# joshbeal/mira

Measured on AMD Instinct MI355X. Metric: bn256_g1_msm_throughput, higher is better.
Workload: dtype u256 mod p (9 x 29-bit limbs in u32/u64, Montgomery)

## Files before the change

mira_amd/csrc/msm_host.cuh:

```cuda
#pragma once
#include "ctx.h"
#ifndef MSM_DIGITS_BLOCK
#define MSM_DIGITS_BLOCK 256
#endif
#include "msm_kernels.cuh"
#include "table_kernels.cuh"
#include "sort_kernels.cuh"
#include "reduce_kernels.cuh"
#include "host_field.hpp"
#include <cerrno>
#include <thread>
#include <unistd.h>

#ifdef MIRA_CPU_EMU
static constexpr uint32_t FIXUP_HEAVY_GRID = 4;
static constexpr uint32_t FIXUP_HEAVY_BLOCKS = 1;
#else
#ifndef MIRA_FIXUP_HEAVY_BLOCKS
#define MIRA_FIXUP_HEAVY_BLOCKS 256
#endif
static constexpr uint32_t FIXUP_HEAVY_BLOCKS = MIRA_FIXUP_HEAVY_BLOCKS;
static constexpr uint32_t FIXUP_HEAVY_GRID = 1024;
#endif

static constexpr uint32_t SCAN_OWN_PREFIX_TILES = 32;
static constexpr uint32_t SCAN_SOLO_TILES = 2;
static inline bool reduce_with_quads(uint64_t work_items) { return work_items * 4 <= 98304; }
#ifdef MIRA_CPU_EMU
static constexpr uint32_t SET_FINISH_BLOCK = 32;
#else
static constexpr uint32_t SET_FINISH_BLOCK = 256;
#endif

static inline std::vector<size_t> host_chunks(size_t n, size_t min_n) {
    std::vector<size_t> ends;
    if (n < min_n) { ends.push_back(n); return ends; }
    size_t done = 0, step = std::max<size_t>(1, min_n / 2);
    while (done < n) {
        size_t len = std::min(step, n - done);
        if (n - done - len < step / 2) len = n - done;
        done += len;
        ends.push_back(done);
        if (step < 4 * std::max<size_t>(1, min_n / 2)) step <<= 1;
    }
    return ends;
}

template <class F, class FS>
static int msm_launch_body(const Bases &bs, size_t first, const void *d_scalars, const void *h_scalars, size_t n, const MsmPlan &p,
                           uint64_t *host_windows );
template <class F, class FS>
static int msm_launch(const Bases &bs, size_t first, const void *d_scalars, const void *h_scalars, size_t n, const MsmPlan &p,
                      uint64_t *host_windows) {
    const uint32_t hist_sel_before = g.hist_sel;
    const int rc = msm_launch_body<F, FS>(bs, first, d_scalars, h_scalars, n, p, host_windows);
    if (rc != MIRA_OK) {
        if (g.copy_stream) (void)rt_sync(g.copy_stream);
        (void)rt_sync(g.stream);
        (void)rt_last();
        if (p.stats && g.hist_dev.p) {
            (void)rt_memset(g.hist_dev.p, 0, 2048, g.stream);
            (void)rt_sync(g.stream);
            g.hist_sel = hist_sel_before;
        }
    }
    return rc;
}
template <class F, class FS>
static int msm_launch_body(const Bases &bs, size_t first, const void *d_scalars, const void *h_scalars, size_t n, const MsmPlan &p,
                           uint64_t *host_windows ) {
    int rc;
    const size_t mult = p.glv ? 2 : 1;
    const size_t host_min = tuned(MIRA_TUNE_HOST_CHUNK_MIN_N, (size_t)1 << 19);
    std::vector<size_t> ends;
    if (h_scalars && p.count == 1) ends = host_chunks(n, host_min);
    else if (p.h_batch) {
        for (size_t e : host_chunks(n * p.count, host_min)) ends.push_back(std::min(n, (e + p.count - 1) / p.count));
        ends.back() = n;
        ends.erase(std::unique(ends.begin(), ends.end()), ends.end());
    } else ends = {n};
    {
        const uint64_t pass_entries = (1ull << tuned(MIRA_TUNE_PASS_ENTRIES_LOG, 32)) - 1;
        const size_t max_chunk = std::max<size_t>(64, (size_t)(pass_entries / ((uint64_t)mult * p.Wt)) / 64 * 64);
        std::vector<size_t> cut;
        for (size_t k = 0, lo = 0; k < ends.size(); lo = ends[k++])
            for (size_t at = lo; at < ends[k];) { at = std::min(ends[k], at + max_chunk); cut.push_back(at); }
        ends.swap(cut);
    }
    size_t nmax = 0;
    for (size_t k = 0, lo = 0; k < ends.size(); lo = ends[k++]) nmax = std::max(nmax, ends[k] - lo);
    nmax *= mult;
    const size_t entries_max = nmax * p.Wt;
    if ((rc = g.digits.ensure(entries_max * 2))) return rc;
    if ((rc = g.counts.ensure(((size_t)p.NB + 1) * 4))) return rc;
    if ((rc = g.offsets.ensure(((size_t)p.NB + 1) * 4))) return rc;
    if ((rc = g.cursor.ensure(((size_t)p.NB + 1) * 4))) return rc;
    const uint32_t scan_blocks = ceil_div(p.NB, SCAN_TILE);
    if (scan_blocks > 1024) { set_error("window configuration exceeds the scan capacity"); return MIRA_E_UNSUPPORTED; }
    if ((rc = g.block_sums.ensure(1024 * 4))) return rc;
    if ((rc = g.sorted_idx.ensure(entries_max * 4 + 8))) return rc;
    const size_t staged_min_n = tuned(MIRA_TUNE_STAGED_MIN_N, (size_t)1 << 19);
    if (nmax * p.count >= staged_min_n && p.c >= 9) {
        if ((rc = g.part.ensure(entries_max * 8 + 8))) return rc;
        if ((rc = g.coarse_offsets.ensure(((size_t)p.Wt * 512 + 1) * 4))) return rc;
    }
    if ((rc = g.bucket_sums.ensure((size_t)p.NB * XYZZ29_BYTES))) return rc;
    if ((rc = g.head_part.ensure((size_t)p.T * XYZZ29_BYTES))) return rc;
    if ((rc = g.tail_part.ensure((size_t)p.T * XYZZ29_BYTES))) return rc;
    if ((rc = g.tail_key.ensure((size_t)p.T * 4))) return rc;
    if ((rc = g.heavy.ensure(64 + ((size_t)p.T / 2 + 8) * 32 + ((size_t)p.T / 4 + 8) * 16))) return rc;
    if ((rc = g.heavy_out.ensure(((size_t)p.T / 2 + 8) * XYZZ29_BYTES))) return rc;
    const size_t node_points = ((size_t)p.nsets << p.gamma) * (p.kappa + 2);
    if ((rc = g.chunks.ensure(node_points * XYZZ29_BYTES))) return rc;
    if ((rc = g.window_sums.ensure((size_t)p.nsets * p.pieces * 128 + 1024))) return rc;
#ifndef MIRA_CPU_EMU
    if (h_scalars || p.h_batch) {
        if (!g.copy_stream) RT_CHECK(hipStreamCreateWithFlags(&g.copy_stream, hipStreamNonBlocking));
        while (g.copy_events.size() < ends.size()) {
            hipEvent_t e;
            RT_CHECK(hipEventCreateWithFlags(&e, hipEventDisableTiming));
            g.copy_events.push_back(e);
        }
    }
#endif

    hipStream_t st = g.stream;
    uint32_t *heavy_count = reinterpret_cast<uint32_t *>(g.heavy.p);
    U4 *heavy_runs = reinterpret_cast<U4 *>(heavy_count + 16);
    U4 *heavy_subs = heavy_runs + ((size_t)p.T / 4 + 4);
    U4 *heavy_meds = reinterpret_cast<U4 *>(reinterpret_cast<unsigned char *>(g.heavy.p) + 64 + ((size_t)p.T / 2 + 8) * 32);
    uint32_t *plan = heavy_count + 2;
    uint32_t *no_u32 = nullptr;
    unsigned char *no_u8 = nullptr;
    const uint32_t fine_bits = (p.c - 1) - std::min<uint32_t>(p.c - 1, 8);
    const uint32_t CB = p.B >> fine_bits;

    tm_begin();
    uint32_t *hist = nullptr, *hist_clear = nullptr;
    if (p.stats) {
        if (!g.hist_dev.p) {
            if ((rc = g.hist_dev.ensure(2048))) return rc;
            RT_CHECK(rt_memset(g.hist_dev.p, 0, 2048, st));
            g.hist_sel = 0;
        }
        hist = reinterpret_cast<uint32_t *>(g.hist_dev.p) + 256 * g.hist_sel;
        hist_clear = reinterpret_cast<uint32_t *>(g.hist_dev.p) + 256 * (g.hist_sel ^ 1u);
        g.hist_sel ^= 1u;
    }
    for (size_t k = 0, lo = 0; k < ends.size(); lo = ends[k++]) {
        const size_t ns = ends[k] - lo, nc = ns * mult, entries = nc * p.Wt;
        const unsigned char *sc = reinterpret_cast<const unsigned char *>(d_scalars) + (p.h_batch ? lo * p.count : lo) * 32;
        const uint64_t stride_k = p.h_batch ? (uint64_t)ns : (uint64_t)p.stride;
        const unsigned char *bases = p.shared ? reinterpret_cast<const unsigned char *>(p.shared_tables)
                                   : p.glv  ? reinterpret_cast<const unsigned char *>(p.glv_bases) + (first + lo) * 128
                                            : reinterpret_cast<const unsigned char *>(bs.d) + (first + lo) * 64;
        const uint32_t wgroup = p.shared ? p.W : 1u, idx_stride = p.shared ? (uint32_t)p.table_n : 0u, idx_first = p.shared ? (uint32_t)(first + lo) : 0u;
        const uint32_t add = k ? 1u : 0u;
        if (h_scalars || p.h_batch) {
            hipStream_t cs = g.copy_stream ? g.copy_stream : st;
            if (p.h_batch)
                for (uint32_t b = 0; b < p.count; b++)
                    RT_CHECK(rt_h2d(const_cast<unsigned char *>(sc) + (size_t)b * ns * 32, reinterpret_cast<const unsigned char *>(p.h_batch[b]) + lo * 32, ns * 32, cs));
            else
                RT_CHECK(rt_h2d(const_cast<unsigned char *>(sc), reinterpret_cast<const unsigned char *>(h_scalars) + lo * 32, ns * 32, cs));
            if (cs != st) RT_CHECK(rt_stream_wait(st, cs, g.copy_events[k]));
        }
        const uint32_t tile = (std::max<uint32_t>(1024, ceil_div(nc, std::max<uint32_t>(1, MSM_HIST_WGS / p.Wt))) + 1023) / 1024 * 1024, ntiles = ceil_div(nc, tile);
        const bool staged = nc * p.count >= staged_min_n && p.c >= 9;
        if (p.glv)
            LAUNCH((k_digits<FS, true>), dim3(ceil_div(ns, MSM_DIGITS_BLOCK), p.count), MSM_DIGITS_BLOCK, 0, st, sc, (uint32_t)ns, stride_k, p.c, p.W,
                   reinterpret_cast<int16_t *>(g.digits.p), reinterpret_cast<uint32_t *>(g.counts.p), p.NB + 1, hist, hist_clear);
        else
        LAUNCH(k_digits<FS>, dim3(ceil_div(nc, MSM_DIGITS_BLOCK), p.count), MSM_DIGITS_BLOCK, 0, st, sc, (uint32_t)nc, stride_k, p.c, p.W,
               reinterpret_cast<int16_t *>(g.digits.p), reinterpret_cast<uint32_t *>(g.counts.p), p.NB + 1, hist, hist_clear);
        tm_mark("digits");
        LAUNCH_BARRIER_FLEX(k_hist, dim3(ntiles, p.Wt), 1024, (size_t)p.B * 4, st, reinterpret_cast<const int16_t *>(g.digits.p), (uint32_t)nc,
                       p.B, tile, reinterpret_cast<uint32_t *>(g.counts.p), wgroup);
        tm_mark("hist");
        if (scan_blocks <= SCAN_SOLO_TILES) {
            LAUNCH_BARRIER(k_scan_c<SCAN_SOLO>, 1, SCAN_BLOCK, 0, st, reinterpret_cast<const uint32_t *>(g.counts.p), p.NB,
                           reinterpret_cast<const uint32_t *>(g.block_sums.p), reinterpret_cast<uint32_t *>(g.offsets.p),
                           reinterpret_cast<uint32_t *>(g.cursor.p), staged ? reinterpret_cast<uint32_t *>(g.coarse_offsets.p) : no_u32, fine_bits,
                           plan, p.lanes, p.L, heavy_count, add ? no_u8 : reinterpret_cast<unsigned char *>(g.bucket_sums.p));
        } else if (scan_blocks <= SCAN_OWN_PREFIX_TILES) {
            LAUNCH_BARRIER(k_scan_c<SCAN_OWN_PREFIX>, scan_blocks, SCAN_BLOCK, 0, st, reinterpret_cast<const uint32_t *>(g.counts.p), p.NB,
                           reinterpret_cast<const uint32_t *>(g.block_sums.p), reinterpret_cast<uint32_t *>(g.offsets.p),
                           reinterpret_cast<uint32_t *>(g.cursor.p), staged ? reinterpret_cast<uint32_t *>(g.coarse_offsets.p) : no_u32, fine_bits,
                           plan, p.lanes, p.L, heavy_count, add ? no_u8 : reinterpret_cast<unsigned char *>(g.bucket_sums.p));
        } else {
        LAUNCH_BARRIER(k_scan_a, scan_blocks, SCAN_BLOCK, 0, st, reinterpret_cast<const uint32_t *>(g.counts.p), p.NB,
                       reinterpret_cast<uint32_t *>(g.block_sums.p));
        LAUNCH_BARRIER(k_scan_b, 1, 1024, 0, st, reinterpret_cast<uint32_t *>(g.block_sums.p), scan_blocks);
        LAUNCH_BARRIER(k_scan_c<SCAN_BLOCK_SUMS>, scan_blocks, SCAN_BLOCK, 0, st, reinterpret_cast<const uint32_t *>(g.counts.p), p.NB,
                       reinterpret_cast<const uint32_t *>(g.block_sums.p), reinterpret_cast<uint32_t *>(g.offsets.p),
                       reinterpret_cast<uint32_t *>(g.cursor.p), staged ? reinterpret_cast<uint32_t *>(g.coarse_offsets.p) : no_u32, fine_bits,
                       plan, p.lanes, p.L, heavy_count, add ? no_u8 : reinterpret_cast<unsigned char *>(g.bucket_sums.p));
        }
        tm_mark("scan");
        if (staged) {
            if (p.shared)
                LAUNCH_BARRIER((k_stage1<int16_t, true, STAGE_TILE_PW>), dim3(ceil_div(nc, STAGE_TILE_PW), p.Wt), 1024, (size_t)STAGE_TILE_PW * 8, st, reinterpret_cast<const int16_t *>(g.digits.p),
                                    (uint32_t)nc, p.B, fine_bits, CB, idx_stride, idx_first, wgroup, reinterpret_cast<uint32_t *>(g.coarse_offsets.p), reinterpret_cast<U2 *>(g.part.p));
            else
                LAUNCH_BARRIER((k_stage1<int16_t, false, STAGE_TILE_PW>), dim3(ceil_div(nc, STAGE_TILE_PW), p.Wt), 1024, (size_t)STAGE_TILE_PW * 8, st, reinterpret_cast<const int16_t *>(g.digits.p),
                                    (uint32_t)nc, p.B, fine_bits, CB, 0u, 0u, 1u, reinterpret_cast<uint32_t *>(g.coarse_offsets.p), reinterpret_cast<U2 *>(g.part.p));
            tm_mark("sort_level1");
            LAUNCH_BARRIER((k_stage2<STAGE_TILE_PW, STAGE_MAX_KEYS2_PW>), ceil_div(entries, STAGE_TILE_PW), 1024, (size_t)STAGE_TILE_PW * 6, st, reinterpret_cast<const U2 *>(g.part.p),
                                reinterpret_cast<const uint32_t *>(g.offsets.p) + p.NB, fine_bits, reinterpret_cast<uint32_t *>(g.cursor.p),
                                reinterpret_cast<uint32_t *>(g.sorted_idx.p));
        } else
            LAUNCH_BARRIER_FLEX(k_scatter, dim3(ntiles, p.Wt), 1024, (size_t)p.B * 4, st, reinterpret_cast<const int16_t *>(g.digits.p),
                       (uint32_t)nc, p.B, tile, reinterpret_cast<uint32_t *>(g.cursor.p), reinterpret_cast<uint32_t *>(g.sorted_idx.p), wgroup, idx_stride, idx_first);
        tm_mark("scatter");
        if (add)
            LAUNCH((k_accumulate<F, true>), ceil_div(p.T, 128), 128, 0, st, reinterpret_cast<const uint32_t *>(g.sorted_idx.p),
                   reinterpret_cast<const uint32_t *>(g.offsets.p), p.NB, bases, (const uint32_t *)plan,
                   reinterpret_cast<unsigned char *>(g.bucket_sums.p), reinterpret_cast<unsigned char *>(g.head_part.p),
                   reinterpret_cast<unsigned char *>(g.tail_part.p), reinterpret_cast<uint32_t *>(g.tail_key.p), heavy_count, heavy_runs, heavy_subs, heavy_meds);
        else
            LAUNCH((k_accumulate<F, false>), ceil_div(p.T, 128), 128, 0, st, reinterpret_cast<const uint32_t *>(g.sorted_idx.p),
                   reinterpret_cast<const uint32_t *>(g.offsets.p), p.NB, bases, (const uint32_t *)plan,
                   reinterpret_cast<unsigned char *>(g.bucket_sums.p), reinterpret_cast<unsigned char *>(g.head_part.p),
                   reinterpret_cast<unsigned char *>(g.tail_part.p), reinterpret_cast<uint32_t *>(g.tail_key.p), heavy_count, heavy_runs, heavy_subs, heavy_meds);
        tm_mark("accumulate");
        const uint32_t fix_by_bucket = p.NB < p.T ? p.NB : 0u;
        const uint32_t fix_items = fix_by_bucket ? fix_by_bucket : p.T;
        LAUNCH_BARRIER(k_fixup_all<F>, FIXUP_HEAVY_BLOCKS + ceil_div(fix_items, HEAVY_BLOCK_A / 4), HEAVY_BLOCK_A, 0, st, FIXUP_HEAVY_BLOCKS, (const uint32_t *)plan,
                       reinterpret_cast<const uint32_t *>(g.offsets.p), reinterpret_cast<const unsigned char *>(g.head_part.p), reinterpret_cast<const unsigned char *>(g.tail_part.p),
                       reinterpret_cast<const uint32_t *>(g.tail_key.p), reinterpret_cast<unsigned char *>(g.bucket_sums.p), fix_by_bucket,
                       (const uint32_t *)heavy_count, (const U4 *)heavy_subs, (const U4 *)heavy_runs, reinterpret_cast<unsigned char *>(g.heavy_out.p), (const U4 *)heavy_meds);
        LAUNCH_BARRIER(k_fixup_heavy_b<F>, (FIXUP_HEAVY_GRID + 3) / 4, HEAVY_BLOCK_B, 0, st, (const uint32_t *)heavy_count, (const U4 *)heavy_runs,
                       reinterpret_cast<const unsigned char *>(g.heavy_out.p), reinterpret_cast<const unsigned char *>(g.tail_part.p),
                       reinterpret_cast<unsigned char *>(g.bucket_sums.p));
        tm_mark("fixup");
    }
    PieceCfg pc;
    pc.P = p.pieces;
    for (uint32_t i = 0; i <= 8; i++) pc.start[i] = piece_start(p.cb, p.pieces, std::min(i, p.pieces));
    const uint32_t tree_groups = p.nsets << p.gamma, npts = p.nsets * p.pieces;
    const size_t lds_a = ((size_t)2 << p.kappa) * XYZZ29_BYTES, lds_b = ((size_t)(p.kappa + 2) << p.gamma) * XYZZ29_BYTES;
    if (p.rquad)
        LAUNCH_BARRIER((k_bucket_tree<F, true>), tree_groups, std::max(4u, 4u << p.kappa), lds_a, st, reinterpret_cast<const unsigned char *>(g.bucket_sums.p),
                       p.lambda, p.kappa, reinterpret_cast<unsigned char *>(g.chunks.p));
    else
        LAUNCH_BARRIER((k_bucket_tree<F, false>), tree_groups, std::max(4u, 1u << p.kappa), lds_a, st, reinterpret_cast<const unsigned char *>(g.bucket_sums.p),
                       p.lambda, p.kappa, reinterpret_cast<unsigned char *>(g.chunks.p));
    tm_mark("reduce_chunks");
    uint32_t *no_ctr = nullptr;
    uint64_t *no_flag = nullptr;
    if (g.windows_dst) {
        LAUNCH_BARRIER(k_set_finish<F>, p.nsets, SET_FINISH_BLOCK, lds_b, st, reinterpret_cast<const unsigned char *>(g.chunks.p), p.kappa + 2, p.gamma, p.lambda, pc,
                       reinterpret_cast<unsigned char *>(g.window_sums.p), (const uint32_t *)hist, no_ctr, no_flag, (uint64_t)0);
        tm_mark("window_sum");
        RT_CHECK(rt_last());
        RT_CHECK(rt_d2d(g.windows_dst, g.window_sums.p, (size_t)npts * 128, st));
        RT_CHECK(rt_sync(st));
    } else {
        const size_t bytes = (size_t)npts * 128 + 1024, flag_at = (bytes + 63) / 64 * 64;
        if (g.out_host_cap < flag_at + 64) {
            RT_CHECK(rt_sync(st));
            if (g.out_host) (void)rt_host_free(g.out_host);
            g.out_host = g.out_host_dev = nullptr; g.out_host_cap = 0;
            RT_CHECK(rt_host_alloc_mapped(reinterpret_cast<void **>(&g.out_host), reinterpret_cast<void **>(&g.out_host_dev), flag_at + 64 + 4096));
            g.out_host_cap = flag_at + 64 + 4096;
        }
        if (!g.finish_ctr.p) {
            if ((rc = g.finish_ctr.ensure(64))) return rc;
            RT_CHECK(rt_memset(g.finish_ctr.p, 0, 64, st));
        }
        uint64_t *flag_host = reinterpret_cast<uint64_t *>(g.out_host + flag_at);
        const uint64_t stamp = ++g.out_stamp;
        __atomic_store_n(flag_host, (uint64_t)0, __ATOMIC_RELEASE);
        LAUNCH_BARRIER(k_set_finish<F>, p.nsets, SET_FINISH_BLOCK, lds_b, st, reinterpret_cast<const unsigned char *>(g.chunks.p), p.kappa + 2, p.gamma, p.lambda, pc,
                       g.out_host_dev, (const uint32_t *)hist, reinterpret_cast<uint32_t *>(g.finish_ctr.p), reinterpret_cast<uint64_t *>(g.out_host_dev + flag_at), stamp);
        tm_mark("window_sum");
        RT_CHECK(rt_last());
        if (g.tm.enabled || (size_t)n * p.count > ((size_t)1 << 21)) RT_CHECK(rt_sync(st));
        RT_CHECK(rt_wait_flag(flag_host, stamp, st));
        memcpy(host_windows, g.out_host, (size_t)npts * 128);
        if (p.stats) memcpy(g.hist_host, g.out_host + (size_t)npts * 128, 1024);
    }
    tm_end();
    return MIRA_OK;
}


template <class F, class FS> static int curve_init() {
#ifndef MIRA_CPU_EMU
    RT_CHECK(hipFuncSetAttribute(reinterpret_cast<const void *>(k_window_sum<F, false>), hipFuncAttributeMaxDynamicSharedMemorySize, 160 * 1024));
    RT_CHECK(hipFuncSetAttribute(reinterpret_cast<const void *>(k_bucket_tree<F, true>), hipFuncAttributeMaxDynamicSharedMemorySize, 160 * 1024));
    RT_CHECK(hipFuncSetAttribute(reinterpret_cast<const void *>(k_bucket_tree<F, false>), hipFuncAttributeMaxDynamicSharedMemorySize, 160 * 1024));
    RT_CHECK(hipFuncSetAttribute(reinterpret_cast<const void *>(k_set_finish<F>), hipFuncAttributeMaxDynamicSharedMemorySize, 160 * 1024));
    RT_CHECK(hipFuncSetAttribute(reinterpret_cast<const void *>(k_hist), hipFuncAttributeMaxDynamicSharedMemorySize, 160 * 1024));
    RT_CHECK(hipFuncSetAttribute(reinterpret_cast<const void *>(k_scatter), hipFuncAttributeMaxDynamicSharedMemorySize, 160 * 1024));
    RT_CHECK(hipFuncSetAttribute(reinterpret_cast<const void *>(k_stage1<int16_t, false, STAGE_TILE_PW>), hipFuncAttributeMaxDynamicSharedMemorySize, STAGE_TILE_PW * 8));
    RT_CHECK(hipFuncSetAttribute(reinterpret_cast<const void *>(k_stage1<int32_t, true>), hipFuncAttributeMaxDynamicSharedMemorySize, STAGE_TILE * 8));
    RT_CHECK(hipFuncSetAttribute(reinterpret_cast<const void *>(k_stage1<int16_t, true, STAGE_TILE_PW>), hipFuncAttributeMaxDynamicSharedMemorySize, STAGE_TILE_PW * 8));
    RT_CHECK(hipFuncSetAttribute(reinterpret_cast<const void *>(k_stage2<STAGE_TILE, STAGE_MAX_KEYS2>), hipFuncAttributeMaxDynamicSharedMemorySize, STAGE_TILE * 6));
    RT_CHECK(hipFuncSetAttribute(reinterpret_cast<const void *>(k_stage2<STAGE_TILE_PW, STAGE_MAX_KEYS2_PW>), hipFuncAttributeMaxDynamicSharedMemorySize, STAGE_TILE_PW * 6));
#endif
    return MIRA_OK;
}
template <class FS> static int synth_scalars(size_t n, uint64_t index0, uint64_t seed, int kind, void *d_out) {
    LAUNCH(k_synth_scalars<FS>, ceil_div(n, 256), 256, 0, g.stream, (uint64_t)n, index0, seed, kind, reinterpret_cast<unsigned char *>(d_out));
    RT_CHECK(rt_last());
    RT_CHECK(rt_sync(g.stream));
    return MIRA_OK;
}
template <class FB, int CURVE> static int synth_bases(size_t n, uint64_t index0, uint64_t seed, void *d_out) {
    LAUNCH(k_synth_bases<FB>, ceil_div(n, 64), 64, 0, g.stream, (uint64_t)n, index0, seed, reinterpret_cast<const unsigned char *>(dev_consts()->gen[CURVE]),
           reinterpret_cast<unsigned char *>(d_out));
    RT_CHECK(rt_last());
    RT_CHECK(rt_sync(g.stream));
    return MIRA_OK;
}
template <class F, int CURVE> static int check_bases(const Bases &bs, uint32_t *d_bad) {
    LAUNCH(k_check_on_curve<F>, ceil_div(bs.n, 256), 256, 0, g.stream, (const unsigned char *)bs.d, (uint64_t)bs.n,
           reinterpret_cast<const unsigned char *>(dev_consts()->b_r261[CURVE]), d_bad);
    RT_CHECK(rt_last());
    return MIRA_OK;
}
template <class F> static int convert_bases(const void *d_src, void *d_dst, size_t n) {
    if (!n) return MIRA_OK;
    LAUNCH(k_convert_bases<F>, ceil_div(n, 256), 256, 0, g.stream, reinterpret_cast<const unsigned char *>(d_src),
           reinterpret_cast<unsigned char *>(d_dst), (uint64_t)n);
    RT_CHECK(rt_last());
    RT_CHECK(rt_sync(g.stream));
    return MIRA_OK;
}
template <class F> static int export_bases(const Bases &bs, size_t first, size_t n, void *d_out) {
    if (!n) return MIRA_OK;
    LAUNCH(k_export_bases<F>, ceil_div(n, 256), 256, 0, g.stream, reinterpret_cast<const unsigned char *>(bs.d) + first * 64,
           reinterpret_cast<unsigned char *>(d_out), (uint64_t)n);
    RT_CHECK(rt_last());
    RT_CHECK(rt_sync(g.stream));
    return MIRA_OK;
}

template <class F, int CURVE> static int build_glv(Bases &bs) {
    const size_t bytes = (size_t)bs.n * 128;
    void *t = nullptr;
    if (rt_malloc(&t, bytes) != hipSuccess || !t) {
        set_error("device allocation of " + std::to_string(bytes) + " bytes for the endomorphism copy of the key failed");
        return MIRA_E_ALLOC;
    }
    LAUNCH(k_glv_bases<F>, ceil_div(bs.n, 256), 256, 0, g.stream, reinterpret_cast<const unsigned char *>(bs.d), reinterpret_cast<unsigned char *>(t), (uint64_t)bs.n,
           reinterpret_cast<const unsigned char *>(dev_consts()->beta_r261[CURVE]));
    if (rt_last() != hipSuccess || rt_sync(g.stream) != hipSuccess) { (void)rt_free(t); set_error("building the endomorphism copy of the key failed"); return MIRA_E_NO_DEVICE; }
    bs.glv = t;
    return MIRA_OK;
}

template <class F> static int build_tables(Bases &bs, uint32_t c, uint32_t W) {
    if (bs.tables || bs.n == 0) return MIRA_OK;
    const size_t bytes = (size_t)W * bs.n * 64;
    void *t = nullptr;
    if (rt_malloc(&t, bytes) != hipSuccess || !t) {
        set_error("device allocation of " + std::to_string(bytes) + " bytes for the window tables failed");
        return MIRA_E_ALLOC;
    }
    unsigned char *tb = reinterpret_cast<unsigned char *>(t);
    RT_CHECK(rt_d2d(tb, bs.d, bs.n * 64, g.stream));
    for (uint32_t w = 1; w < W; w++)
        LAUNCH(k_table_step<F>, ceil_div(bs.n, 64), 64, 0, g.stream, (const unsigned char *)(tb + (size_t)(w - 1) * bs.n * 64),
               tb + (size_t)w * bs.n * 64, (uint64_t)bs.n, c);
    RT_CHECK(rt_last());
    RT_CHECK(rt_sync(g.stream));
    bs.tables = t; bs.table_c = c; bs.table_w = W;
    return MIRA_OK;
}

template <class F, class FS>
static int msm_launch_table(const Bases &bs, size_t first, const void *d_scalars, size_t n, uint64_t *host_sums) {
    int rc;
    const TableCfg tc = table_cfg(bs.table_c);
    const uint32_t TABLE_W = tc.W, TABLE_B = tc.B, TABLE_FINE_BITS = tc.fine_bits;
    const size_t entries = (size_t)n * TABLE_W;
    const uint32_t lanes = 256u * 4u * 3u * 64u, Lmin = 16;
    const uint32_t T = (uint32_t)std::min<uint64_t>(lanes, ceil_div(entries, Lmin));
    const uint32_t m = 8, nchunks = TABLE_B / m;
    if ((rc = g.digits.ensure(entries * 4))) return rc;
    if ((rc = g.counts.ensure(((size_t)TABLE_CB + 1) * 4))) return rc;
    if ((rc = g.coarse_offsets.ensure(((size_t)TABLE_CB + 1) * 4))) return rc;
    if ((rc = g.cursor.ensure(((size_t)TABLE_CB + 1) * 4))) return rc;
    if ((rc = g.block_sums.ensure(1024 * 4))) return rc;
    if ((rc = g.part.ensure(entries * 8 + 8))) return rc;
    if ((rc = g.sorted_idx.ensure(entries * 4 + 8))) return rc;
    if ((rc = g.offsets.ensure(((size_t)TABLE_B + 1) * 4))) return rc;
    if ((rc = g.fine_counts.ensure(((size_t)TABLE_B + 1) * 4))) return rc;
    if ((rc = g.fine_cursor.ensure(((size_t)TABLE_B + 1) * 4))) return rc;
    if ((rc = g.bucket_sums.ensure((size_t)TABLE_B * XYZZ29_BYTES))) return rc;
    if ((rc = g.head_part.ensure((size_t)T * XYZZ29_BYTES))) return rc;
    if ((rc = g.tail_part.ensure((size_t)T * XYZZ29_BYTES))) return rc;
    if ((rc = g.tail_key.ensure((size_t)T * 4))) return rc;
    if ((rc = g.heavy.ensure(64 + ((size_t)T / 2 + 8) * 32 + ((size_t)T / 4 + 8) * 16))) return rc;
    if ((rc = g.heavy_out.ensure(((size_t)T / 2 + 8) * XYZZ29_BYTES))) return rc;
    if ((rc = g.chunks.ensure((size_t)nchunks * XYZZ29_BYTES))) return rc;
    if ((rc = g.window_sums.ensure((size_t)TABLE_SUMS * 128))) return rc;

    hipStream_t st = g.stream;
    uint32_t *heavy_count = reinterpret_cast<uint32_t *>(g.heavy.p);
    uint32_t *plan = heavy_count + 2;
    U4 *heavy_runs = reinterpret_cast<U4 *>(heavy_count + 16);
    U4 *heavy_subs = heavy_runs + ((size_t)T / 4 + 4);
    U4 *heavy_meds = reinterpret_cast<U4 *>(reinterpret_cast<unsigned char *>(g.heavy.p) + 64 + ((size_t)T / 2 + 8) * 32);
    const uint32_t tile = 32768, ntiles = ceil_div(n, tile);
    tm_begin();
    uint32_t *no_u32 = nullptr;
    unsigned char *no_u8 = nullptr;
    RT_CHECK(rt_memset(g.counts.p, 0, ((size_t)TABLE_CB + 1) * 4, st));
    tm_mark("memset");
    LAUNCH(k_digits32<FS>, ceil_div(n, 256), 256, 0, st, reinterpret_cast<const unsigned char *>(d_scalars), (uint32_t)n, tc.c, tc.W,
           reinterpret_cast<int32_t *>(g.digits.p));
    tm_mark("digits");
    LAUNCH_BARRIER_FLEX(k_thist_coarse, dim3(ntiles, TABLE_W), 512, 0, st, reinterpret_cast<const int32_t *>(g.digits.p), (uint32_t)n, tile, TABLE_FINE_BITS,
                        reinterpret_cast<uint32_t *>(g.counts.p));
    tm_mark("hist");
    LAUNCH_BARRIER(k_scan_a, 1, SCAN_BLOCK, 0, st, reinterpret_cast<const uint32_t *>(g.counts.p), TABLE_CB, reinterpret_cast<uint32_t *>(g.block_sums.p));
    LAUNCH_BARRIER(k_scan_b, 1, 1024, 0, st, reinterpret_cast<uint32_t *>(g.block_sums.p), 1u);
    LAUNCH_BARRIER(k_scan_c<SCAN_BLOCK_SUMS>, 1, SCAN_BLOCK, 0, st, reinterpret_cast<const uint32_t *>(g.counts.p), TABLE_CB,
                   reinterpret_cast<const uint32_t *>(g.block_sums.p), reinterpret_cast<uint32_t *>(g.coarse_offsets.p),
                   reinterpret_cast<uint32_t *>(g.cursor.p), no_u32, 0u, no_u32, 0u, 0u, no_u32, no_u8);
    tm_mark("scan");
    const uint32_t *coarse_total = reinterpret_cast<const uint32_t *>(g.coarse_offsets.p) + TABLE_CB;
    LAUNCH_BARRIER((k_stage1<int32_t, true>), dim3(ceil_div(n, STAGE_TILE), TABLE_W), 1024, (size_t)STAGE_TILE * 8, st,
                        reinterpret_cast<const int32_t *>(g.digits.p), (uint32_t)n, TABLE_B, TABLE_FINE_BITS, TABLE_CB, (uint32_t)bs.n, (uint32_t)first, TABLE_W,
                        reinterpret_cast<uint32_t *>(g.cursor.p), reinterpret_cast<U2 *>(g.part.p));
    tm_mark("sort_level1");
    RT_CHECK(rt_memset(g.fine_counts.p, 0, ((size_t)TABLE_B + 1) * 4, st));
    LAUNCH_BARRIER_FLEX(k_stage2_count, ceil_div(entries, STAGE_TILE), 1024, 0, st, reinterpret_cast<const U2 *>(g.part.p), coarse_total, TABLE_FINE_BITS,
                        reinterpret_cast<uint32_t *>(g.fine_counts.p));
    const uint32_t fscan = ceil_div(TABLE_B, SCAN_TILE);
    LAUNCH_BARRIER(k_scan_a, fscan, SCAN_BLOCK, 0, st, reinterpret_cast<const uint32_t *>(g.fine_counts.p), TABLE_B, reinterpret_cast<uint32_t *>(g.block_sums.p));
    LAUNCH_BARRIER(k_scan_b, 1, 1024, 0, st, reinterpret_cast<uint32_t *>(g.block_sums.p), fscan);
    LAUNCH_BARRIER(k_scan_c<SCAN_BLOCK_SUMS>, fscan, SCAN_BLOCK, 0, st, reinterpret_cast<const uint32_t *>(g.fine_counts.p), TABLE_B,
                   reinterpret_cast<const uint32_t *>(g.block_sums.p), reinterpret_cast<uint32_t *>(g.offsets.p), reinterpret_cast<uint32_t *>(g.fine_cursor.p),
                   no_u32, 0u, plan, lanes, Lmin, heavy_count, reinterpret_cast<unsigned char *>(g.bucket_sums.p));
    tm_mark("bucket_count_scan");
    LAUNCH_BARRIER((k_stage2<STAGE_TILE, STAGE_MAX_KEYS2>), ceil_div(entries, STAGE_TILE), 1024, (size_t)STAGE_TILE * 6, st, reinterpret_cast<const U2 *>(g.part.p), coarse_total,
                        TABLE_FINE_BITS, reinterpret_cast<uint32_t *>(g.fine_cursor.p), reinterpret_cast<uint32_t *>(g.sorted_idx.p));
    tm_mark("sort_level2");
    LAUNCH((k_accumulate<F, false>), ceil_div(T, 128), 128, 0, st, reinterpret_cast<const uint32_t *>(g.sorted_idx.p),
           reinterpret_cast<const uint32_t *>(g.offsets.p), TABLE_B, reinterpret_cast<const unsigned char *>(bs.tables), (const uint32_t *)plan,
           reinterpret_cast<unsigned char *>(g.bucket_sums.p), reinterpret_cast<unsigned char *>(g.head_part.p),
           reinterpret_cast<unsigned char *>(g.tail_part.p), reinterpret_cast<uint32_t *>(g.tail_key.p), heavy_count, heavy_runs, heavy_subs, heavy_meds);
    tm_mark("accumulate");
    LAUNCH_BARRIER(k_fixup_all<F>, FIXUP_HEAVY_BLOCKS + ceil_div(T, HEAVY_BLOCK_A / 4), HEAVY_BLOCK_A, 0, st, FIXUP_HEAVY_BLOCKS, (const uint32_t *)plan,
                   reinterpret_cast<const uint32_t *>(g.offsets.p), reinterpret_cast<const unsigned char *>(g.head_part.p), reinterpret_cast<const unsigned char *>(g.tail_part.p),
                   reinterpret_cast<const uint32_t *>(g.tail_key.p), reinterpret_cast<unsigned char *>(g.bucket_sums.p), 0u,
                   (const uint32_t *)heavy_count, (const U4 *)heavy_subs, (const U4 *)heavy_runs, reinterpret_cast<unsigned char *>(g.heavy_out.p), (const U4 *)heavy_meds);
    LAUNCH_BARRIER(k_fixup_heavy_b<F>, (FIXUP_HEAVY_GRID + 3) / 4, HEAVY_BLOCK_B, 0, st, (const uint32_t *)heavy_count, (const U4 *)heavy_runs,
                   reinterpret_cast<const unsigned char *>(g.heavy_out.p), reinterpret_cast<const unsigned char *>(g.tail_part.p),
                   reinterpret_cast<unsigned char *>(g.bucket_sums.p));
    tm_mark("fixup");
    LAUNCH((k_reduce_chunks<F, false>), ceil_div(nchunks, 256), 256, 0, st, reinterpret_cast<const unsigned char *>(g.bucket_sums.p),
           TABLE_B, m, 1u, reinterpret_cast<unsigned char *>(g.chunks.p));
    tm_mark("reduce_chunks");
    LAUNCH_BARRIER((k_window_sum<F, false>), TABLE_SUMS, WSUM_BLOCK, (size_t)WSUM_BLOCK * XYZZ29_BYTES, st,
                   reinterpret_cast<const unsigned char *>(g.chunks.p), nchunks / TABLE_SUMS, reinterpret_cast<unsigned char *>(g.window_sums.p), (const uint32_t *)nullptr);
    tm_mark("window_sum");
    RT_CHECK(rt_last());
    if (g.windows_dst) RT_CHECK(rt_d2d(g.windows_dst, g.window_sums.p, (size_t)TABLE_SUMS * 128, st));
    else RT_CHECK(rt_d2h(host_sums, g.window_sums.p, (size_t)TABLE_SUMS * 128, st));
    RT_CHECK(rt_sync(st));
    tm_end();
    return MIRA_OK;
}

static constexpr size_t KEYFILE_CHUNK_POINTS = (size_t)1 << 20;
static inline int read_exact_parallel(int fd, unsigned char *dst, size_t bytes, size_t file_off) {
    const size_t nthreads = std::max<size_t>(1, std::min<size_t>(8, std::thread::hardware_concurrency()));
    const size_t slice = (bytes + nthreads - 1) / nthreads;
    std::vector<int> fail(nthreads, 0);
    std::vector<std::thread> th;
    auto work = [&](size_t t) {
        size_t lo = std::min(bytes, t * slice), hi = std::min(bytes, lo + slice);
        while (lo < hi) {
            const ssize_t r = pread(fd, dst + lo, hi - lo, (off_t)(file_off + lo));
            if (r <= 0) { fail[t] = 1; return; }
            lo += (size_t)r;
        }
    };
    for (size_t t = 1; t < nthreads; t++) th.emplace_back(work, t);
    work(0);
    for (auto &x : th) x.join();
    for (int f : fail) if (f) return 1;
    return 0;
}
template <class F, int CURVE> static int load_bases_file(Bases &b, int fd, bool validate, uint32_t *d_bad) {
    const unsigned char *d_curve_b = reinterpret_cast<const unsigned char *>(dev_consts()->b_r261[CURVE]);
    unsigned char *pinned[2] = {nullptr, nullptr};
    const size_t chunk_bytes = std::min(b.n, KEYFILE_CHUNK_POINTS) * 64;
    auto body = [&]() -> int {
        for (int k = 0; k < 2; k++) RT_CHECK(rt_host_alloc(reinterpret_cast<void **>(&pinned[k]), chunk_bytes));
#ifndef MIRA_CPU_EMU
        if (!g.copy_stream) RT_CHECK(hipStreamCreateWithFlags(&g.copy_stream, hipStreamNonBlocking));
        while (g.copy_events.size() < 2) {
            hipEvent_t e;
            RT_CHECK(hipEventCreateWithFlags(&e, hipEventDisableTiming));
            g.copy_events.push_back(e);
        }
#endif
        hipStream_t st = g.stream, cs = g.copy_stream ? g.copy_stream : st;
        if (validate) RT_CHECK(rt_memset(d_bad, 0, 4, st));
        unsigned char *dst = reinterpret_cast<unsigned char *>(b.d);
        size_t i = 0;
        for (size_t off = 0; off < b.n; off += KEYFILE_CHUNK_POINTS, i++) {
            const size_t cnt = std::min(KEYFILE_CHUNK_POINTS, b.n - off);
            unsigned char *buf = pinned[i & 1];
#ifndef MIRA_CPU_EMU
            if (i >= 2) RT_CHECK(rt_event_sync(g.copy_events[i & 1]));
#endif
            if (read_exact_parallel(fd, buf, cnt * 64, off * 64)) { set_error("failed to fill whole buffer"); return MIRA_E_IO; }
            RT_CHECK(rt_h2d(dst + off * 64, buf, cnt * 64, cs));
#ifndef MIRA_CPU_EMU
            if (cs != st) RT_CHECK(rt_stream_wait(st, cs, g.copy_events[i & 1]));
            else RT_CHECK(hipEventRecord(g.copy_events[i & 1], cs));
#endif
            LAUNCH(k_convert_bases<F>, ceil_div(cnt, 256), 256, 0, st, (const unsigned char *)(dst + off * 64), dst + off * 64, (uint64_t)cnt);
            if (validate) LAUNCH(k_check_on_curve<F>, ceil_div(cnt, 256), 256, 0, st, (const unsigned char *)(dst + off * 64), (uint64_t)cnt, d_curve_b, d_bad);
        }
        RT_CHECK(rt_last());
        RT_CHECK(rt_sync(cs));
        RT_CHECK(rt_sync(st));
        return MIRA_OK;
// ... 34 lines not shown
```

mira_amd/csrc/msm_kernels.cuh:

```cuda
#pragma once
#include "curve.cuh"
#include "curve29.cuh"
#include "quad29.cuh"
#include "glv.cuh"

static constexpr uint32_t KEY_NONE = 0xFFFFFFFFu;
static constexpr int HEAVY_SPAN = 6;
static constexpr int MEDIUM_SPAN = 12;
#ifdef MIRA_CPU_EMU
static constexpr uint32_t MEDIUM_AS_CHAINS_FROM = 8;
#else
static constexpr uint32_t MEDIUM_AS_CHAINS_FROM = 1024;
#endif
static constexpr int WSUM_BLOCK = 512;
static constexpr uint32_t HEAVY_SUB = 64;

template <class FS, bool GLV = false>
KERNEL void k_digits(const unsigned char *__restrict__ scalars, uint32_t n, uint64_t stride, uint32_t c, uint32_t W,
                     int16_t *__restrict__ digits, uint32_t *__restrict__ counts, uint32_t ncounts,
                     uint32_t *__restrict__ hist, uint32_t *__restrict__ hist_clear) {
    __shared__ uint32_t bins[256];
    uint32_t i = blockIdx.x * blockDim.x + threadIdx.x;
    for (uint32_t k = (blockIdx.y * gridDim.x + blockIdx.x) * blockDim.x + threadIdx.x; k < ncounts; k += gridDim.x * gridDim.y * blockDim.x) counts[k] = 0;
    const bool sampled = hist && (gridDim.x < 8 || (blockIdx.x & 7u) == 0);
// ... 199 lines not shown
    DYN_SHARED(uint32_t, bins);
    const uint32_t w = blockIdx.y;
    for (uint32_t b = threadIdx.x; b < B; b += blockDim.x) bins[b] = 0;
    __syncthreads();
    const uint32_t base = blockIdx.x * tile, end = (base + tile < n) ? base + tile : n;
    const int16_t *dw = digits + (size_t)w * n;
    for (uint32_t i = base + threadIdx.x; i < end; i += blockDim.x) {
        int32_t d = dw[i];
        if (d != 0) atomicAdd(&bins[(uint32_t)(d < 0 ? -d : d) - 1], 1u);
    }
    __syncthreads();
    for (uint32_t b = threadIdx.x; b < B; b += blockDim.x) {
        uint32_t cnt = bins[b];
        if (cnt) bins[b] = atomicAdd(&cursor[(size_t)(w / wgroup) * B + b], cnt);
    }
    __syncthreads();
    for (uint32_t i = base + threadIdx.x; i < end; i += blockDim.x) {
        int32_t d = dw[i];
        if (d != 0) {
            uint32_t b = (uint32_t)(d < 0 ? -d : d) - 1;
            uint32_t pos = atomicAdd(&bins[b], 1u);
            sorted[pos] = ((w % wgroup) * idx_stride + idx_first + i) | (d < 0 ? 0x80000000u : 0u);
        }
    }
}

template <class F>
KERNEL void k_convert_bases(const unsigned char *__restrict__ src, unsigned char *__restrict__ dst, uint64_t n) {
    using S = typename F::Sat;
    uint64_t i = (uint64_t)blockIdx.x * blockDim.x + threadIdx.x;
    if (i >= n) return;
    Fe<S> x = fe_load<S>(src + i * 64), y = fe_load<S>(src + i * 64 + 32);
    if (!(fe_is_zero(x) && fe_is_zero(y))) {
        x = reduce_once(f29_pack(f29_from_r256<F>(x)));
        y = reduce_once(f29_pack(f29_from_r256<F>(y)));
    }
    fe_store(dst + i * 64, x);
    fe_store(dst + i * 64 + 32, y);
}

template <class F>
KERNEL void k_export_bases(const unsigned char *__restrict__ src, unsigned char *__restrict__ dst, uint64_t n) {
    using S = typename F::Sat;
    uint64_t i = (uint64_t)blockIdx.x * blockDim.x + threadIdx.x;
    if (i >= n) return;
    Fe<S> x = fe_load<S>(src + i * 64), y = fe_load<S>(src + i * 64 + 32);
    if (!(fe_is_zero(x) && fe_is_zero(y))) {
        x = f29_to_r256(f29_unpack_canonical<F>(x));
        y = f29_to_r256(f29_unpack_canonical<F>(y));
    }
    fe_store(dst + i * 64, x);
    fe_store(dst + i * 64 + 32, y);
}

template <class F>
KERNEL void k_check_on_curve(const unsigned char *__restrict__ bases, uint64_t n, const unsigned char *__restrict__ b_r261,
                             uint32_t *__restrict__ bad_count) {
    using S = typename F::Sat;
    uint64_t i = (uint64_t)blockIdx.x * blockDim.x + threadIdx.x;
    if (i >= n) return;
    Aff29<F> p = aff29_load<F>(bases + i * 64, false);
    if (aff29_is_identity(p)) return;
    Fe29<F> lhs = f29_sqr(p.y);
    Fe29<F> rhs = f29_add(f29_mul(f29_sqr(p.x), p.x), f29_unpack_canonical<F>(fe_load<S>(b_r261)));
    if (!f29_is_zero_mod_p<6>(f29_sub<4>(lhs, rhs))) atomicAdd(bad_count, 1u);
}

DEV uint32_t bucket_of(const uint32_t *__restrict__ offsets, uint32_t lo, uint32_t NB, uint32_t pos) {
    uint32_t hi = NB;
    while (hi - lo > 1) {
        uint32_t mid = lo + ((hi - lo) >> 1);
        if (offsets[mid] <= pos) lo = mid; else hi = mid;
    }
    return lo;
}

template <bool ADD, class F> DEV Xyzz29<F> run_start(const unsigned char *bucket_sums, uint32_t bucket) {
    if constexpr (ADD) return xyzz29_load<F>(bucket_sums + (size_t)bucket * XYZZ29_BYTES);
    else return xyzz29_identity<F>();
}
#ifdef MSM_PROBE_STAMPS
static __device__ uint64_t g_acc_stamps[4096 * 3];
#endif
template <class F, bool ADD>
KERNEL void __launch_bounds__(128) __attribute__((amdgpu_waves_per_eu(3, 3))) k_accumulate(const uint32_t *__restrict__ sorted, const uint32_t *__restrict__ offsets, uint32_t NB,
                         const unsigned char *__restrict__ bases,
                         const uint32_t *__restrict__ plan, unsigned char *__restrict__ bucket_sums,
                         unsigned char *__restrict__ head_part, unsigned char *__restrict__ tail_part, uint32_t *__restrict__ tail_key,
                         uint32_t *__restrict__ heavy_ctr, U4 *__restrict__ runs, U4 *__restrict__ subs, U4 *__restrict__ meds) {
    const uint32_t t = blockIdx.x * blockDim.x + threadIdx.x;
#ifdef MSM_PROBE_STAMPS
    const uint64_t probe_t0 = __builtin_amdgcn_s_memrealtime();
#endif
    const uint32_t total = offsets[NB];
    const uint32_t L = plan[0];
    const uint64_t start64 = (uint64_t)t * L;
    if (start64 >= total) return;
    const uint32_t start = (uint32_t)start64;
    const uint32_t end = (total - start > L) ? start + L : total;
    uint32_t cur = bucket_of(offsets, 0, NB, start);
    uint32_t run_end = offsets[cur + 1];
    uint32_t next_end = offsets[cur + 2 <= NB ? cur + 2 : NB];
    const bool cont_prev = offsets[cur] < start;
    bool first = true;
    Xyzz29<F> acc = cont_prev ? xyzz29_identity<F>() : run_start<ADD, F>(bucket_sums, cur);
    uint32_t ent0 = sorted[start];
    uint32_t ent1 = (start + 1 < end) ? sorted[start + 1] : ent0;
    const U4 *bp = reinterpret_cast<const U4 *>(bases + (size_t)(ent0 & 0x7FFFFFFFu) * 64);
    U4 r0 = bp[0], r1 = bp[1], r2 = bp[2], r3 = bp[3];
    for (uint32_t j = start; j < end; j++) {
        const uint32_t e = ent0;
        const U4 c0 = r0, c1 = r1, c2 = r2, c3 = r3;
        bp = reinterpret_cast<const U4 *>(bases + (size_t)(ent1 & 0x7FFFFFFFu) * 64);
        r0 = bp[0]; r1 = bp[1]; r2 = bp[2]; r3 = bp[3];
        ent0 = ent1;
        ent1 = sorted[(j + 2 < end) ? j + 2 : end - 1];
        if (j == run_end) {
            if (first && cont_prev) xyzz29_store(head_part + (size_t)t * XYZZ29_BYTES, acc);
            else xyzz29_store(bucket_sums + (size_t)cur * XYZZ29_BYTES, acc);
            first = false;
            cur++;
            run_end = next_end;
            if (run_end <= j) {
                cur = bucket_of(offsets, cur, NB, j);
                run_end = offsets[cur + 1];
            }
            next_end = offsets[cur + 2 <= NB ? cur + 2 : NB];
            acc = run_start<ADD, F>(bucket_sums, cur);
        }
        xyzz29_add_affine(acc, aff29_from_raw<F>(c0, c1, c2, c3, (e >> 31) != 0));
    }
    const bool cont_next = end < run_end;
    const bool is_head = first && cont_prev;
    if (is_head) xyzz29_store(head_part + (size_t)t * XYZZ29_BYTES, acc);
    else if (cont_next) xyzz29_store(tail_part + (size_t)t * XYZZ29_BYTES, acc);
    else xyzz29_store(bucket_sums + (size_t)cur * XYZZ29_BYTES, acc);
    const bool holds_tail = !is_head && cont_next;
    tail_key[t] = holds_tail ? cur : KEY_NONE;
#ifdef MSM_PROBE_STAMPS
    if ((threadIdx.x & 63u) == 0 && (t >> 6) < 4096u) {
        uint32_t hwid;
        asm volatile("s_getreg_b32 %0, hwreg(HW_REG_HW_ID)" : "=s"(hwid));
        g_acc_stamps[(t >> 6) * 3] = hwid; g_acc_stamps[(t >> 6) * 3 + 1] = probe_t0; g_acc_stamps[(t >> 6) * 3 + 2] = __builtin_amdgcn_s_memrealtime();
    }
#endif
    if (holds_tail) {
        const uint32_t span = (run_end - 1) / L - t;
        if (span > (uint32_t)HEAVY_SPAN && span <= (uint32_t)MEDIUM_SPAN) {
            meds[atomicAdd(&heavy_ctr[5], 1u)] = U4{t, span, cur, 0};
        } else if (span > (uint32_t)MEDIUM_SPAN) {
            const uint32_t nsub = (span + HEAVY_SUB - 1) / HEAVY_SUB;
            const uint32_t h = atomicAdd(&heavy_ctr[0], 1u);
            const uint32_t base = atomicAdd(&heavy_ctr[1], nsub);
            if (nsub > 1) atomicAdd(&heavy_ctr[4], 1u);
            runs[h] = U4{t, span, cur, base};
            for (uint32_t q = 0; q < nsub; q++) {
                const uint32_t first_p = t + 1 + q * HEAVY_SUB;
                const uint32_t cnt = (span - q * HEAVY_SUB < HEAVY_SUB) ? span - q * HEAVY_SUB : HEAVY_SUB;
                subs[base + q] = U4{first_p, cnt, h, 0};
            }
        }
    }
}

template <bool QUAD, class F> DEV void xyzz29_add_sel(Xyzz29<F> &acc, const Xyzz29<F> &q) {
    if constexpr (QUAD) xyzz29_add_quad(acc, q); else xyzz29_add(acc, q);
}
template <bool QUAD, class F> DEV Xyzz29<F> xyzz29_double_sel(const Xyzz29<F> &p) {
    if constexpr (QUAD) return xyzz29_double_quad(p); else return xyzz29_double(p);
}
DEV uint32_t quad_gid() { return (blockIdx.x * blockDim.x + threadIdx.x) >> 2; }

DEV bool medium_as_chains(const uint32_t *__restrict__ heavy_ctr) { return heavy_ctr[5] >= MEDIUM_AS_CHAINS_FROM && heavy_ctr[1] != 0; }
template <class F>
DEV void fixup_chain(uint32_t t, uint32_t span, uint32_t key, const unsigned char *__restrict__ head_part, const unsigned char *__restrict__ tail_part,
                     unsigned char *__restrict__ bucket_sums) {
    Xyzz29<F> acc = xyzz29_load<F>(tail_part + (size_t)t * XYZZ29_BYTES);
    Xyzz29<F> nxt = xyzz29_load<F>(head_part + (size_t)(t + 1) * XYZZ29_BYTES);
    for (uint32_t q = 1; q <= span; q++) {
        const Xyzz29<F> cur = nxt;
        nxt = xyzz29_load<F>(head_part + (size_t)(t + (q < span ? q + 1 : q)) * XYZZ29_BYTES);
        xyzz29_add_quad(acc, cur);
    }
    if (quad_lane() == 0) xyzz29_store(bucket_sums + (size_t)key * XYZZ29_BYTES, acc);
}
template <class F>
DEV void fixup_light(uint32_t gid, uint32_t nquads, const uint32_t *__restrict__ plan, const uint32_t *__restrict__ offsets,
                     const unsigned char *__restrict__ head_part, const unsigned char *__restrict__ tail_part,
                     const uint32_t *__restrict__ tail_key, unsigned char *__restrict__ bucket_sums, uint32_t num_buckets,
                     const uint32_t *__restrict__ heavy_ctr, const U4 *__restrict__ meds) {
    const uint32_t n_medium = heavy_ctr[5];
    if (medium_as_chains(heavy_ctr))
        for (uint32_t m = gid; m < n_medium; m += nquads) {
            const U4 r = meds[m];
            fixup_chain<F>(r.x, r.y, r.z, head_part, tail_part, bucket_sums);
        }
    const uint32_t L = plan[0], T = plan[1];
    uint32_t t, key, run_end;
    if (num_buckets) {
// ... 229 lines not shown
```

Baseline: 685.2.

## Stage sorted indices into LDS via async global_load_lds in accumulate

Each thread in k_accumulate now prefetches its slice of sorted bucket indices into a per-wave double-buffered LDS stage using global_load_lds, instead of issuing a dependent global load per iteration. Index reads in the hot loop come from LDS, and the next 16-entry block is fetched asynchronously. The sorted_idx buffer is padded so the over-reading prefetch stays in bounds. Risks include the waitcnt of zero stalling on all outstanding memory ops including base-point loads, extra LDS use per block, and the per-lane 4-aligned staging assumption.

```diff
diff --git a/mira_amd/csrc/msm_host.cuh b/mira_amd/csrc/msm_host.cuh
--- a/mira_amd/csrc/msm_host.cuh
+++ b/mira_amd/csrc/msm_host.cuh
@@ -98,7 +98,7 @@
     const uint32_t scan_blocks = ceil_div(p.NB, SCAN_TILE);
     if (scan_blocks > 1024) { set_error("window configuration exceeds the scan capacity"); return MIRA_E_UNSUPPORTED; }
     if ((rc = g.block_sums.ensure(1024 * 4))) return rc;
-    if ((rc = g.sorted_idx.ensure(entries_max * 4 + 8))) return rc;
+    if ((rc = g.sorted_idx.ensure(entries_max * 4 + 8 + ACC_STAGE_PAD))) return rc;
     const size_t staged_min_n = tuned(MIRA_TUNE_STAGED_MIN_N, (size_t)1 << 19);
     if (nmax * p.count >= staged_min_n && p.c >= 9) {
         if ((rc = g.part.ensure(entries_max * 8 + 8))) return rc;
@@ -213,12 +213,12 @@
                        (uint32_t)nc, p.B, tile, reinterpret_cast<uint32_t *>(g.cursor.p), reinterpret_cast<uint32_t *>(g.sorted_idx.p), wgroup, idx_stride, idx_first);
         tm_mark("scatter");
         if (add)
-            LAUNCH((k_accumulate<F, true>), ceil_div(p.T, 128), 128, 0, st, reinterpret_cast<const uint32_t *>(g.sorted_idx.p),
+            LAUNCH((k_accumulate<F, true>), ceil_div(p.T, ACC_BLOCK), ACC_BLOCK, 0, st, reinterpret_cast<const uint32_t *>(g.sorted_idx.p),
                    reinterpret_cast<const uint32_t *>(g.offsets.p), p.NB, bases, (const uint32_t *)plan,
                    reinterpret_cast<unsigned char *>(g.bucket_sums.p), reinterpret_cast<unsigned char *>(g.head_part.p),
                    reinterpret_cast<unsigned char *>(g.tail_part.p), reinterpret_cast<uint32_t *>(g.tail_key.p), heavy_count, heavy_runs, heavy_subs, heavy_meds);
         else
-            LAUNCH((k_accumulate<F, false>), ceil_div(p.T, 128), 128, 0, st, reinterpret_cast<const uint32_t *>(g.sorted_idx.p),
+            LAUNCH((k_accumulate<F, false>), ceil_div(p.T, ACC_BLOCK), ACC_BLOCK, 0, st, reinterpret_cast<const uint32_t *>(g.sorted_idx.p),
                    reinterpret_cast<const uint32_t *>(g.offsets.p), p.NB, bases, (const uint32_t *)plan,
                    reinterpret_cast<unsigned char *>(g.bucket_sums.p), reinterpret_cast<unsigned char *>(g.head_part.p),
                    reinterpret_cast<unsigned char *>(g.tail_part.p), reinterpret_cast<uint32_t *>(g.tail_key.p), heavy_count, heavy_runs, heavy_subs, heavy_meds);
@@ -385,7 +385,7 @@
     if ((rc = g.cursor.ensure(((size_t)TABLE_CB + 1) * 4))) return rc;
     if ((rc = g.block_sums.ensure(1024 * 4))) return rc;
     if ((rc = g.part.ensure(entries * 8 + 8))) return rc;
-    if ((rc = g.sorted_idx.ensure(entries * 4 + 8))) return rc;
+    if ((rc = g.sorted_idx.ensure(entries * 4 + 8 + ACC_STAGE_PAD))) return rc;
     if ((rc = g.offsets.ensure(((size_t)TABLE_B + 1) * 4))) return rc;
     if ((rc = g.fine_counts.ensure(((size_t)TABLE_B + 1) * 4))) return rc;
     if ((rc = g.fine_cursor.ensure(((size_t)TABLE_B + 1) * 4))) return rc;
@@ -440,7 +440,7 @@
     LAUNCH_BARRIER((k_stage2<STAGE_TILE, STAGE_MAX_KEYS2>), ceil_div(entries, STAGE_TILE), 1024, (size_t)STAGE_TILE * 6, st, reinterpret_cast<const U2 *>(g.part.p), coarse_total,
                         TABLE_FINE_BITS, reinterpret_cast<uint32_t *>(g.fine_cursor.p), reinterpret_cast<uint32_t *>(g.sorted_idx.p));
     tm_mark("sort_level2");
-    LAUNCH((k_accumulate<F, false>), ceil_div(T, 128), 128, 0, st, reinterpret_cast<const uint32_t *>(g.sorted_idx.p),
+    LAUNCH((k_accumulate<F, false>), ceil_div(T, ACC_BLOCK), ACC_BLOCK, 0, st, reinterpret_cast<const uint32_t *>(g.sorted_idx.p),
            reinterpret_cast<const uint32_t *>(g.offsets.p), TABLE_B, reinterpret_cast<const unsigned char *>(bs.tables), (const uint32_t *)plan,
            reinterpret_cast<unsigned char *>(g.bucket_sums.p), reinterpret_cast<unsigned char *>(g.head_part.p),
            reinterpret_cast<unsigned char *>(g.tail_part.p), reinterpret_cast<uint32_t *>(g.tail_key.p), heavy_count, heavy_runs, heavy_subs, heavy_meds);
diff --git a/mira_amd/csrc/msm_kernels.cuh b/mira_amd/csrc/msm_kernels.cuh
--- a/mira_amd/csrc/msm_kernels.cuh
+++ b/mira_amd/csrc/msm_kernels.cuh
@@ -305,12 +305,45 @@
 #ifdef MSM_PROBE_STAMPS
 static __device__ uint64_t g_acc_stamps[4096 * 3];
 #endif
+#ifndef MSM_ACC_STAGE
+#define MSM_ACC_STAGE 1
+#endif
+static constexpr uint32_t ACC_BLOCK = 128, ACC_STAGE = 16, ACC_STAGE_PAD = ACC_STAGE * 4;
+static constexpr uint32_t ACC_STAGE_WAVE_WORDS = 2 * 64 * ACC_STAGE;
+DEV uint32_t acc_lane() { return threadIdx.x & 63u; }
+#ifdef MIRA_CPU_EMU
+DEV uint32_t acc_wave() { return threadIdx.x >> 6; }
+#else
+DEV uint32_t acc_wave() { return __builtin_amdgcn_readfirstlane(threadIdx.x >> 6); }
+#endif
+DEV void acc_stage_block(uint32_t *wave_stage, uint32_t buf, const uint32_t *src) {
+#ifdef MIRA_CPU_EMU
+    for (uint32_t q = 0; q < ACC_STAGE / 4; q++) memcpy(wave_stage + buf * (64 * ACC_STAGE) + q * 256 + acc_lane() * 4, src + 4 * q, 16);
+#else
+    uint32_t *dst = wave_stage + __builtin_amdgcn_readfirstlane(buf) * (64 * ACC_STAGE);
+#pragma unroll
+    for (uint32_t q = 0; q < ACC_STAGE / 4; q++)
+        __builtin_amdgcn_global_load_lds((__attribute__((address_space(1))) void *)(src + 4 * q),
+                                         (__attribute__((address_space(3))) void *)(dst + q * 256), 16, 0, 0);
+#endif
+}
+DEV uint32_t acc_staged(const uint32_t *wave_stage, uint32_t r) {
+    return wave_stage[((r / ACC_STAGE) & 1u) * (64 * ACC_STAGE) + ((r % ACC_STAGE) >> 2) * 256 + acc_lane() * 4 + (r & 3u)];
+}
+DEV void acc_stage_wait() {
+#ifndef MIRA_CPU_EMU
+    __builtin_amdgcn_s_waitcnt(0x0F70);
+#endif
+}
 template <class F, bool ADD>
-KERNEL void __launch_bounds__(128) __attribute__((amdgpu_waves_per_eu(3, 3))) k_accumulate(const uint32_t *__restrict__ sorted, const uint32_t *__restrict__ offsets, uint32_t NB,
+KERNEL void __launch_bounds__(ACC_BLOCK) __attribute__((amdgpu_waves_per_eu(3, 3))) k_accumulate(const uint32_t *__restrict__ sorted, const uint32_t *__restrict__ offsets, uint32_t NB,
                          const unsigned char *__restrict__ bases,
                          const uint32_t *__restrict__ plan, unsigned char *__restrict__ bucket_sums,
                          unsigned char *__restrict__ head_part, unsigned char *__restrict__ tail_part, uint32_t *__restrict__ tail_key,
                          uint32_t *__restrict__ heavy_ctr, U4 *__restrict__ runs, U4 *__restrict__ subs, U4 *__restrict__ meds) {
+#if MSM_ACC_STAGE
+    __shared__ __attribute__((aligned(16))) uint32_t stage[(ACC_BLOCK / 64) * ACC_STAGE_WAVE_WORDS];
+#endif
     const uint32_t t = blockIdx.x * blockDim.x + threadIdx.x;
 #ifdef MSM_PROBE_STAMPS
     const uint64_t probe_t0 = __builtin_amdgcn_s_memrealtime();
@@ -329,15 +362,33 @@
     Xyzz29<F> acc = cont_prev ? xyzz29_identity<F>() : run_start<ADD, F>(bucket_sums, cur);
     uint32_t ent0 = sorted[start];
     uint32_t ent1 = (start + 1 < end) ? sorted[start + 1] : ent0;
+#if MSM_ACC_STAGE
+    uint32_t *wave_stage = stage + acc_wave() * ACC_STAGE_WAVE_WORDS;
+    const uint32_t stage_at = start & ~3u;
+    acc_stage_block(wave_stage, 0, sorted + stage_at);
+    if (stage_at + ACC_STAGE < end) acc_stage_block(wave_stage, 1, sorted + stage_at + ACC_STAGE);
+#endif
     const U4 *bp = reinterpret_cast<const U4 *>(bases + (size_t)(ent0 & 0x7FFFFFFFu) * 64);
     U4 r0 = bp[0], r1 = bp[1], r2 = bp[2], r3 = bp[3];
     for (uint32_t j = start; j < end; j++) {
+#if MSM_ACC_STAGE
+        acc_stage_wait();
+#endif
         const uint32_t e = ent0;
         const U4 c0 = r0, c1 = r1, c2 = r2, c3 = r3;
         bp = reinterpret_cast<const U4 *>(bases + (size_t)(ent1 & 0x7FFFFFFFu) * 64);
         r0 = bp[0]; r1 = bp[1]; r2 = bp[2]; r3 = bp[3];
         ent0 = ent1;
+#if MSM_ACC_STAGE
+        {
+            const uint32_t r = ((j + 2 < end) ? j + 2 : end - 1) - stage_at;
+            ent1 = acc_staged(wave_stage, r);
+            if (r % ACC_STAGE == 0 && stage_at + r + ACC_STAGE < end)
+                acc_stage_block(wave_stage, (r / ACC_STAGE + 1) & 1u, sorted + stage_at + r + ACC_STAGE);
+        }
+#else
         ent1 = sorted[(j + 2 < end) ? j + 2 : end - 1];
+#endif
         if (j == run_end) {
             if (first && cont_prev) xyzz29_store(head_part + (size_t)t * XYZZ29_BYTES, acc);
             else xyzz29_store(bucket_sums + (size_t)cur * XYZZ29_BYTES, acc);
```

Measured after the change: 703.6, median of 6. 2.7% higher.
